# cbg-ethz/metMHN

Measured on AMD Instinct MI355X. Metric: full-cohort log-lik+grad evals/sec at n=20 events; kronvec HBM GB/s, higher is better.
Workload: dtype f64

## Files before the change

metmhn_amd/csrc/engine.hip:

```cpp
#include <algorithm>
#include <chrono>
#include <cmath>
#include <cstdio>
#include <cstdlib>
#include <cstring>
#include <string>
#include <vector>

#include "../../include/metmhn_amd.h"
#include "host.h"
#include "comm.h"
#include "plan.h"
#include "sampler.h"

namespace mmhn {

static thread_local std::string g_err;

struct CListDev {
  DevArr<CItem> items;
  DevArr<int> deps;
};
struct StagedDev {
  DevArr<int> pats, paired, probs;
// ... 14 lines not shown
};

struct Config {
  PlanCfg plan;
  bool zero_copy = true;
  bool poison = false;
  bool force_timing = false;
  bool coop_fault = false;
  int coop_wgs = 0;
  bool coop = true;
  long long sim_chunk = 1ll << 26;
  int stream_blocks = 256 * 8;
  bool trace_host = false;
  Config() {
    plan.use_jacobi = env_is("MMHN_SOLVER", "jacobi");
    plan.psolve_min = (int)env_int("MMHN_PSOLVE_MIN", plan.psolve_min);
    plan.wsolve_min = (int)env_int("MMHN_WSOLVE_MIN", env_set("MMHN_PSOLVE_MIN") ? plan.psolve_min : plan.wsolve_min);
    plan.wsolve_mode = (int)env_int("MMHN_WSOLVE", plan.wsolve_mode);
    plan.wsolve_wgs = (int)env_int("MMHN_WSOLVE_WGS", plan.wsolve_wgs);
    plan.prep_split_max = (int)env_int("MMHN_PREP_SPLIT", plan.prep_split_max);
    plan.pcl_per = std::max(1, (int)env_int("MMHN_PCL_PER", plan.pcl_per));
    plan.small_path = env_flag("MMHN_SMALL", plan.small_path);
    zero_copy = env_flag("MMHN_ZEROCOPY", zero_copy);
    poison = env_flag("MMHN_POISON", poison);
    force_timing = env_flag("MMHN_TIME_KERNELS", force_timing);
    coop_fault = env_flag("MMHN_COOP_FAULT", coop_fault);
    coop_wgs = (int)env_int("MMHN_COOP_WGS", coop_wgs);
    coop = env_flag("MMHN_COOP", coop);
    sim_chunk = std::max(1ll, env_int("MMHN_SIM_CHUNK", sim_chunk));
    stream_blocks = (int)env_int("MMHN_STREAM_BLOCKS", stream_blocks);
    trace_host = env_set("MMHN_TRACE_HOST");
  }
};

struct EngineBase {
  virtual ~EngineBase() = default;
  int dtype = 0;
  int device = 0;
  hipStream_t stream = nullptr;
  Config cfg;
};

template <typename T>
struct PList {
  const Desc* d; const int2* map; int ntiles; int maxk; long long vec;
  const int2* lmap; const std::vector<int>* lof; const T* tab;
  const CList* cl = nullptr;
  const CListDev* dcl = nullptr;
  int kslot = MMHN_K_OTHER_SOLVE;
};

template <typename... K>
static void raise_lds(size_t bytes, K... kernels) {
  for (const void* k : {reinterpret_cast<const void*>(kernels)...})
    HIPCHECK(hipFuncSetAttribute(k, hipFuncAttributeMaxDynamicSharedMemorySize, (int)bytes));
}

template <typename T>
struct Engine : EngineBase {
  using PList = mmhn::PList<T>;
  int n = 0, N = 0;
  DevArr<Params<T>> d_par;
  Params<T>* h_par = nullptr;
  void* h_par_dev = nullptr;
  DevArr<uint16_t> d_perm;
  DevArr<int> d_lvl;
  std::vector<int8_t> dat;
  long long n_pat = 0;
  int n_cols = 0;
  double n_em = 0;
  std::vector<Batch> batches;
  std::vector<BatchDev> dev;
  DevArr<T> pi, lidgJ, qJ, rhsJ, rhsS, pS, lidgS, qS, seedS, GS, dots, bmJ, bmS, tabJ, tabS;
  DevArr<T> piM, qM;
  DevArr<T> zarena;
  struct View { T* p = nullptr; } GJ, DJ, Abuf;
  int pi_owner = -1, qJ_owner = -1;
  DevArr<double> lp, out, sums, abi_sums, redbuf;
  DevArr<JLink<T>> links;
  double* h_abi = nullptr;
  double* h_abi_dev = nullptr;
  hipStream_t side[3] = {};
  hipEvent_t ev_fork[3] = {}, ev_join[3] = {};
  bool small_forked[2] = {false, false}, fork_recorded[2] = {false, false};
  DevArr<CoopCtl> coop_ctl;
  DevArr<unsigned> coop_flags[2];
  unsigned coop_epoch = 0;
  int coop_slot = 0;
  int cur_lane = 0;
  unsigned* h_abort = nullptr;
  unsigned* h_abort_dev = nullptr;
  bool coop_used = false;
  bool coop_alone = false;
  bool sums_pending = false;
  std::chrono::steady_clock::time_point sums_t0, sums_issued;
  int sums_len = 0;
  int pack_mode = 0;
  double pack_a = 0, pack_b = 0;
  double* pack_dst = nullptr;
  bool packed_in_eval = false;
  double reduce_flag = 0.0, reduce_flag_sum = 0.0;
  bool flag_pending = false;
  ncclComm_t comm = nullptr;
  int comm_rank = 0, comm_size = 1;
  bool time_kernels = true;
  mmhn_counters cnt{};
  std::vector<std::pair<hipEvent_t, hipEvent_t>> ev_pool;
  size_t ev_used = 0;
  std::vector<double> ev_bytes;
  std::vector<int> ev_slot;

  static long long zarena_elems(long long nJ, long long asize, int N) { return up4(3 * nJ * N * N) + up4(3 * nJ * N) + up4(asize); }
  static long long zclear_elems(const Batch& b, int N) { return zarena_elems((long long)b.dJ.size(), b.aclr, N); }

  Engine(int dev_id, int n_mut) : n(n_mut), N(n_mut + 1) {
    device = dev_id;
    cnt.comm_rank = -1;
    REQUIRE(n_mut >= 1 && n_mut < MAXN, "n_mut must be in [1, 31]");
    DevGuard guard(device);
    HIPCHECK(hipStreamCreateWithFlags(&stream, hipStreamNonBlocking));
    d_par.alloc(NPSET);
    HIPCHECK(hipHostMalloc(reinterpret_cast<void**>(&h_par), NPSET * sizeof(Params<T>), hipHostMallocDefault));
    HIPCHECK(hipHostGetDevicePointer(&h_par_dev, h_par, 0));
    static_assert(sizeof(Params<T>) % sizeof(uint4) == 0, "parameter block: whole 16-byte words");
    sums.alloc(2 * stride());
    size_t free_b = 0, total_b = 0;
    HIPCHECK(hipMemGetInfo(&free_b, &total_b));
    cfg.plan.ws_limit = (size_t)(0.7 * (double)free_b);
    hipDeviceProp_t prop;
    HIPCHECK(hipGetDeviceProperties(&prop, device));
    cfg.plan.n_cu = std::max(1, prop.multiProcessorCount);
    {
      std::vector<uint16_t> perm((size_t)(TB + 1) << TB, 0);
      std::vector<int> lvl((size_t)(TB + 1) * (TB + 2), 0);
      for (int t = 0; t <= TB; ++t) {
        int pos = 0;
        for (int l = 0; l <= t; ++l) {
          lvl[(size_t)t * (TB + 2) + l] = pos;
          for (uint32_t x = 0; x < (1u << t); ++x)
            if (popc(x) == l) perm[((size_t)t << TB) + pos++] = (uint16_t)x;
        }
        lvl[(size_t)t * (TB + 2) + t + 1] = pos;
      }
      d_perm.alloc(perm.size());
      d_lvl.alloc(lvl.size());
      HIPCHECK(hipMemcpy(d_perm.p, perm.data(), perm.size() * sizeof(uint16_t), hipMemcpyHostToDevice));
      HIPCHECK(hipMemcpy(d_lvl.p, lvl.data(), lvl.size() * sizeof(int), hipMemcpyHostToDevice));
    }
    raise_lds(wsolve_lds<T>(), &k_wsolve<T, false>, &k_wsolve<T, true>, &k_wsolve<T, false, WCfg<T>::NXT>, &k_wsolve<T, true, WCfg<T>::NXT>);
    raise_lds(wclass_lds<T>(), &k_wclass<T>);
    raise_lds(160 * 1024, &k_spatient2<T>, &k_spatient<T, 1024, 1>);
    raise_lds(150 * 1024,
              &k_csolve<T, false, false>, &k_csolve<T, true, false>, &k_csolve<T, false, true>, &k_csolve<T, true, true>,
              &k_csolve<T, false, false, 4>, &k_csolve<T, true, false, 4>,
              &k_psolve2<T, false, true>, &k_psolve2<T, true, true>, &k_psolve2<T, false, false>, &k_psolve2<T, true, false>,
              &k_tsolve<T, false, false>, &k_tsolve<T, true, false>, &k_tsolve<T, false, true>, &k_tsolve<T, true, true>,
              &k_kv<T, false, 1, false>, &k_kv<T, true, 1, false>, &k_kv<T, false, 1, true>, &k_kv<T, true, 1, true>,
              &k_sweep<T, false>, &k_sweep<T, true>, &k_diag<T>, &k_diag<T, 1024>,
              &k_prep<T, false>, &k_prep<T, true>, &k_prep<T, false, 1024>, &k_grad_rows<T, 1>, &k_grad_rows<T>,
              &k_pclass<T, false>, &k_pclass<T, true>, &k_class_marg<T>);
    coop_ctl.alloc(1);
    HIPCHECK(hipMemset(coop_ctl.p, 0, sizeof(CoopCtl)));
    HIPCHECK(hipHostMalloc(reinterpret_cast<void**>(&h_abort), 64, hipHostMallocDefault));
    HIPCHECK(hipHostGetDevicePointer(reinterpret_cast<void**>(&h_abort_dev), h_abort, 0));
    *h_abort = 0u;
    for (int i = 0; i < 3; ++i) {
      HIPCHECK(hipStreamCreateWithFlags(&side[i], hipStreamNonBlocking));
      HIPCHECK(hipEventCreateWithFlags(&ev_fork[i], hipEventDisableTiming));
      HIPCHECK(hipEventCreateWithFlags(&ev_join[i], hipEventDisableTiming));
    }
  }
  ~Engine() override {
    comm_destroy();
    for (auto& e : ev_pool) { (void)hipEventDestroy(e.first); (void)hipEventDestroy(e.second); }
    for (int i = 0; i < 3; ++i) {
      if (ev_join[i]) (void)hipEventDestroy(ev_join[i]);
      if (ev_fork[i]) (void)hipEventDestroy(ev_fork[i]);
      if (side[i]) (void)hipStreamDestroy(side[i]);
    }
    if (h_par) (void)hipHostFree(h_par);
    if (h_abi) (void)hipHostFree(h_abi);
    if (h_abort) (void)hipHostFree(h_abort);
    if (stream) (void)hipStreamDestroy(stream);
    stream = nullptr;
  }
  int stride() const { return 1 + N * N + 2 * N; }

  void build_params(const double* lt, const double* ldp, const double* ldm, bool upload = true) {
    REQUIRE(!sums_pending, "an evaluation begun with mmhn_cohort_sums_begin has not been collected (its parameter upload may still be in flight)");
    std::vector<double> eth((size_t)N * N), enp(N, 1.0), enm(N, 1.0);
    for (int e = 0; e < N * N; ++e) eth[e] = std::exp(lt[e]);
    if (ldp) for (int j = 0; j < N; ++j) enp[j] = std::exp(-ldp[j]);
    if (ldm) for (int j = 0; j < N; ++j) enm[j] = std::exp(-ldm[j]);
    for (int s = 0; s < NPSET; ++s) {
      Params<T>& P = h_par[s];
      std::memset(&P, 0, sizeof(P));
      for (int i = 0; i < N; ++i) {
        for (int j = 0; j < N; ++j) {
          double v = eth[i * N + j];
          if (s == PS_PRIM && j == n && i < n) v = 1.0;
          if (s == PS_MET && i != j) v *= enm[j];
          if (s == PS_PRIM && i != j) v *= enp[j];
          P.th[i][j] = (T)v;
        }
        P.baseP[i] = (T)eth[i * N + i];
        P.baseM[i] = i < n ? (T)(eth[i * N + i] * eth[i * N + n]) : (T)0;
        P.dp[i] = (T)(ldp ? std::exp(ldp[i]) : 1.0);
        P.dm[i] = (T)(ldm ? std::exp(ldm[i]) : 1.0);
      }
    }
    if (!upload) return;
    if (cfg.zero_copy) {
      const int nw = (int)(NPSET * sizeof(Params<T>) / sizeof(uint4));
      hipLaunchKernelGGL(k_copy_words, dim3((nw + 255) / 256), dim3(256), 0, stream, static_cast<const uint4*>(h_par_dev),
                         reinterpret_cast<uint4*>(d_par.p), nw);
      HIPCHECK(hipGetLastError());
    } else {
      HIPCHECK(hipMemcpyAsync(d_par.p, h_par, NPSET * sizeof(Params<T>), hipMemcpyHostToDevice, stream));
    }
  }

  size_t sweep_lds(int maxk) const { return DESC_PAD + ((size_t)(1 << TB) + 2 * (size_t)std::max(maxk, 1) * 64) * sizeof(T); }
  void prep(const Desc* descs, int nprob, T* tab, bool joint = false, int maxkc = 0) {
    if (nprob == 0) return;
    const int parts = maxkc > 9 ? 1 << std::min(maxkc - 9, 5) : 1;
    if (joint && nprob <= cfg.plan.prep_split_max) hipLaunchKernelGGL((k_prep<T, true>), dim3(nprob, 4 * parts), dim3(BLOCK), prep_lds<T>(N), stream, descs, d_par.p, tab);
    else if (nprob >= 256) hipLaunchKernelGGL((k_prep<T, false, 1024>), dim3(nprob), dim3(1024), prep_lds<T>(N), stream, descs, d_par.p, tab);
    else hipLaunchKernelGGL((k_prep<T, false>), dim3(nprob), dim3(BLOCK), prep_lds<T>(N), stream, descs, d_par.p, tab);
    HIPCHECK(hipGetLastError());
  }

  void launch_sweep(bool tr, const Desc* descs, const int2* map, int ntiles, int maxk, const T* p, T* y,
                    const T* lidg, const T* rhs, int rhs_mode, const T* scal, double alg_bytes, const T* tab) {
    if (ntiles == 0) return;
    const size_t lds = sweep_lds(maxk);
    auto launch = [&]() {
      if (tr)
        hipLaunchKernelGGL((k_sweep<T, true>), dim3(ntiles), dim3(KSB), lds, stream, descs, map, d_par.p, p, y,
                           lidg, rhs, rhs_mode, scal, std::max(maxk, 1), tab);
      else
        hipLaunchKernelGGL((k_sweep<T, false>), dim3(ntiles), dim3(KSB), lds, stream, descs, map, d_par.p, p, y,
                           lidg, rhs, rhs_mode, scal, std::max(maxk, 1), tab);
    };
    if (alg_bytes > 0) { timed(MMHN_K_OTHER_SOLVE, alg_bytes, launch); return; }
    launch();
    HIPCHECK(hipGetLastError());
  }
  void launch_kv(bool tr, const Desc* descs, const int2* map, int ntiles, int maxk, const T* p, T* y, const T* tab, const T* hxt,
                 const int* zmap = nullptr, const T* lidg = nullptr, const T* rhs = nullptr) {
    if (ntiles == 0) return;
    const size_t lds = DESC_PAD + ((size_t)(1 << TB) + 2 * (size_t)maxk * 64 + 32) * sizeof(T);
#define KV_ARGS dim3(ntiles), dim3(KSB), lds, stream, descs, map, ntiles, p, y, tab, hxt, maxk, zmap, lidg, rhs
    if (lidg) {
      if (tr) hipLaunchKernelGGL((k_kv<T, true, 1, true>), KV_ARGS);
      else hipLaunchKernelGGL((k_kv<T, false, 1, true>), KV_ARGS);
    } else {
      if (tr) hipLaunchKernelGGL((k_kv<T, true, 1, false>), KV_ARGS);
// ... 248 lines not shown
    links.alloc(std::max<size_t>(mnJ, 1));
    tabJ.alloc(mtJ); tabS.alloc(mtS);
    pi_owner = qJ_owner = -1;
    rhsS.alloc(mvS); pS.alloc(mvS); lidgS.alloc(mvS); qS.alloc(mvS);
    seedS.alloc(mnS);
    GS.alloc(mnS * N * N); zarena.alloc(mZ);
    dots.alloc(2 * mp); bmJ.alloc(mnJ * 64); bmS.alloc(mnS * 64);
    lp.alloc(mp); out.alloc(mp * stride()); redbuf.alloc(((mp + red_per((int)mp) - 1) / red_per((int)mp)) * 2 * (size_t)stride());
  }

  void small_fork(int which) {
    HIPCHECK(hipEventRecord(ev_fork[which], stream));
    fork_recorded[which] = true;
  }
  void small_classes(const Batch& b, int which, bool grad) {
    const BatchDev& db = dev[b.id];
    const int n0 = (int)b.sp_list[which][0].size(), n1 = (int)b.sp_list[which][1].size(), n2 = (int)b.sp_list[which][2].size();
    const int np0 = which ? (int)b.sp_list[2][0].size() : 0, np1 = which ? (int)b.sp_list[2][1].size() : 0;
    const int mk0 = spatient_class_maxk(0), mk1 = which ? b.mk1p : spatient_class_maxk(1), mk2 = spatient_class_maxk(2);
    const bool on_side = which == 0 ? (n0 + n1 + n2 > 0) : n2 > 0;
    hipStream_t sd = side[which];
    if (on_side) {
      if (!fork_recorded[which]) HIPCHECK(hipEventRecord(ev_fork[which], stream));
      HIPCHECK(hipStreamWaitEvent(sd, ev_fork[which], 0));
    }
    fork_recorded[which] = false;
#define SP_TAIL db.pats.p, db.dS.p, d_par.p, d_perm.p, d_lvl.p, db.dJ.p, db.wd.p, pi.p, links.p, pS.p, qS.p, GS.p, bmS.p, dots.p, lp.p
    auto big_class = [&]() {
      if (!n2) return;
      const size_t lds = (spatient_lds<T>(N, mk2) + 15) / 16 * 16;
      hipLaunchKernelGGL((k_spatient<T, 1024, 1>), dim3(n2), dim3(1024), lds, sd, db.sp_list[which][2].p, n2, SP_TAIL, mk2, N, grad ? 1 : 0);
      HIPCHECK(hipGetLastError());
    };
    big_class();
    if (n0 + n1 + np0 + np1) {
      const size_t s0 = (spatient_lds<T>(N, mk0) + 15) / 16 * 16, s1 = (spatient_lds<T>(N, mk1) + 15) / 16 * 16;
      const size_t lds = std::max(s0 * SP_PPB0, n1 + np1 ? s1 * (np1 ? 2 : 1) : 0) + 64;
      const int nblk = (n0 + SP_PPB0 - 1) / SP_PPB0 + n1 + (np0 + SP_PPB0 / 2 - 1) / (SP_PPB0 / 2) + np1;
      hipLaunchKernelGGL((k_spatient2<T>), dim3(nblk), dim3(256), lds, which == 0 ? sd : stream,
                         db.sp_list[which][0].p, n0, mk0, db.sp_list[which][1].p, n1, mk1,
                         db.sp_list[2][0].p, np0, db.sp_list[2][1].p, np1, SP_TAIL, N, grad ? 1 : 0);
      HIPCHECK(hipGetLastError());
    }
#undef SP_TAIL
    if (on_side) HIPCHECK(hipEventRecord(ev_join[which], sd));
    small_forked[which] = on_side;
  }
  void small_join(int which) {
    if (small_forked[which]) HIPCHECK(hipStreamWaitEvent(stream, ev_join[which], 0));
    small_forked[which] = false;
  }

  void evaluate(const double* lt, const double* ldp, const double* ldm, bool grad, double* host_sums,
                double* host_out) {
    REQUIRE(!sums_pending, "an evaluation begun with mmhn_cohort_sums_begin has not been collected");
    auto t0 = std::chrono::steady_clock::now();
    const int st = stride();
    small_forked[0] = small_forked[1] = fork_recorded[0] = fork_recorded[1] = false;
    bool head_done = false;
    if (cfg.zero_copy && !batches.empty()) {
      build_params(lt, ldp, ldm, false);
      const Batch& b0 = batches.front();
      long long nz = grad && !b0.dJ.empty() ? zclear_elems(b0, N) * (long long)sizeof(T) / 16 : 0;
      const bool fill_here = nz <= (32ll << 20) / 16;
      if (!fill_here) nz = 0;
      const int nw = (int)(NPSET * sizeof(Params<T>) / sizeof(uint4));
      const long long need = std::max<long long>(std::max<long long>(nw, 2 * st), nz);
      const int nblk = (int)std::min<long long>((need + 255) / 256, 4096);
      hipLaunchKernelGGL(k_begin_eval, dim3(nblk), dim3(256), 0, stream, static_cast<const uint4*>(h_par_dev),
                         reinterpret_cast<uint4*>(d_par.p), nw, sums.p, 2 * st, reinterpret_cast<uint4*>(zarena.p), nz);
      HIPCHECK(hipGetLastError());
      head_done = fill_here;
    } else {
      build_params(lt, ldp, ldm);
      HIPCHECK(hipMemsetAsync(sums.p, 0, 2 * st * sizeof(double), stream));
    }
    for (const Batch& b : batches) {
      const BatchDev& db = dev[b.id];
      const int npat = (int)b.pats.size(), nJ = (int)b.dJ.size(), nS = (int)b.dS.size();
      const int tJ = (int)b.mapJ.size();
      const PList LJ{db.dJ.p, db.mapJ.p, tJ, b.maxkJ, b.vecJ, db.lmapJ.p, &b.lofJ, tabJ.p};
      const bool fused_small = b.has_small;
      coop_alone = b.stg[0].empty();
      auto staged_fwd = [&](int w) {
        const Staged& g = b.stg[w];
        const StagedDev& dg = db.stg[w];
        if (g.empty()) return;
        const int nG = (int)g.pats.size(), tG = (int)g.map.size();
        const PList LG{db.dS.p, dg.map.p, tG, g.maxk, b.vecS, dg.lmap.p, &g.lof, tabS.p, g.cl, dg.cl};
        hipLaunchKernelGGL((k_staged_init<T>), dim3(nG), dim3(BLOCK), 0, stream, db.pats.p, db.dS.p, rhsS.p, GS.p, bmS.p, N, grad ? 1 : 0, dg.pats.p);
        HIPCHECK(hipGetLastError());
        if (g.probs.size() >= 256)
          hipLaunchKernelGGL((k_prep<T, false, 1024>), dim3((unsigned)g.probs.size()), dim3(1024), prep_lds<T>(N), stream, db.dS.p, d_par.p, tabS.p, dg.probs.p);
        else
          hipLaunchKernelGGL((k_prep<T, false>), dim3((unsigned)g.probs.size()), dim3(BLOCK), prep_lds<T>(N), stream, db.dS.p, d_par.p, tabS.p, dg.probs.p);
        HIPCHECK(hipGetLastError());
        if (!g.paired.empty()) {
          hipLaunchKernelGGL((k_gather_marg<T>), dim3((unsigned)g.paired.size(), 2, g.maxk > 10 ? 8 : 1), dim3(BLOCK), 0, stream,
                             db.pats.p, db.dJ.p, db.dS.p, d_par.p, pi.p, rhsS.p, links.p, dg.paired.p, db.wd.p);
          HIPCHECK(hipGetLastError());
        }
        launch_diag(db.dS.p, dg.map.p, tG, nullptr, lidgS.p, nullptr, KD_LIDG);
        solve(false, LG, pS.p, lidgS.p, rhsS.p, 0, nullptr);
        hipLaunchKernelGGL((k_seeds<T>), dim3((nG + 255) / 256), dim3(256), 0, stream, db.pats.p, nG, db.dS.p,
                           d_par.p, pS.p, seedS.p, lp.p, dg.pats.p);
        HIPCHECK(hipGetLastError());
      };
      auto staged_adj = [&](int w) {
        const Staged& g = b.stg[w];
        const StagedDev& dg = db.stg[w];
        if (g.empty()) return;
        const int tG = (int)g.map.size();
        const PList LG{db.dS.p, dg.map.p, tG, g.maxk, b.vecS, dg.lmap.p, &g.lof, tabS.p, g.cl, dg.cl};
        solve(true, LG, qS.p, lidgS.p, nullptr, 1, seedS.p);
        launch_grad_rows(db.dS.p, (int)g.probs.size(), g.maxk, nullptr, pS.p, qS.p, GS.p, GK_S, dg.grc);
        if (g.kind2) {
          hipLaunchKernelGGL((k_bit_marg<T>), dim3(tG), dim3(BLOCK), 0, stream, db.dS.p, dg.map.p, d_par.p, pS.p, qS.p, bmS.p);
          HIPCHECK(hipGetLastError());
        }
      };
      time_kernels = cfg.force_timing || b.vecJ + b.vecS >= (1ll << 26);
      const long long gjs = (long long)nJ * N * N;
      GJ.p = zarena.p;
      DJ.p = GJ.p + up4(3 * gjs);
      Abuf.p = DJ.p + up4(3ll * nJ * N);
      if (grad && nJ && !(head_done && &b == &batches.front())) zero(zarena.p, zclear_elems(b, N));
      if (grad && nJ && cfg.poison) poison_fill(Abuf.p + b.aclr, b.asize - b.aclr);
      prep(db.dJ.p, nJ, tabJ.p, true, b.maxkcJ);
      bool own_forked = false;
      if (!b.stg[0].empty() && !time_kernels) {
        HIPCHECK(hipEventRecord(ev_fork[2], stream));
        HIPCHECK(hipStreamWaitEvent(side[2], ev_fork[2], 0));
        hipStream_t keep = stream;
        stream = side[2]; cur_lane = 1;
        try {
          staged_fwd(0);
          if (grad) staged_adj(0);
        } catch (...) { stream = keep; cur_lane = 0; throw; }
        stream = keep; cur_lane = 0;
        HIPCHECK(hipEventRecord(ev_join[2], side[2]));
        own_forked = true;
      }
      if (fused_small) small_fork(0);
      if (!cfg.plan.use_jacobi && nJ) {
        if (pi_owner != b.id) { zero(pi.p + b.offT, b.vecJ - b.offT); pi_owner = b.id; }
        if (grad && qJ_owner != b.id) { zero(qJ.p + b.offT, b.vecJ - b.offT); qJ_owner = b.id; }
        if (cfg.poison && b.offT > 0) {
          HIPCHECK(hipMemsetAsync(pi.p, 0xFF, (size_t)b.offT * sizeof(T), stream));
          if (grad) HIPCHECK(hipMemsetAsync(qJ.p, 0xFF, (size_t)b.offT * sizeof(T), stream));
        }
      }
      if (cfg.plan.use_jacobi) {
        launch_diag(db.dJ.p, db.mapJ.p, tJ, nullptr, lidgJ.p, nullptr, KD_LIDG);
        solve(false, LJ, pi.p, lidgJ.p, nullptr, 2, nullptr);
      } else {
        psolve(false, b, pi.p, 2);
      }
      if (fused_small) small_classes(b, 0, grad);
      if (fused_small) small_classes(b, 1, grad);
      if (!own_forked) staged_fwd(0);
      staged_fwd(1);
      if (grad) {
        if (!own_forked) staged_adj(0);
        staged_adj(1);
        small_join(1);
        if (nJ) {
          if (cfg.plan.use_jacobi) zero(rhsJ.p, b.vecJ);
          for (int part = 0; part < 2 && !b.stg[1].paired.empty(); ++part) {
            if (b.stg[1].paired.size() >= 256)
              hipLaunchKernelGGL((k_scatter_marg<T, 1024>), dim3((unsigned)b.stg[1].paired.size()), dim3(1024), 0, stream, db.pats.p, db.dJ.p,
                                 db.dS.p, d_par.p, qS.p, rhsS.p, cfg.plan.use_jacobi ? rhsJ.p : nullptr, dots.p, part, db.stg[1].paired.p);
            else
            hipLaunchKernelGGL((k_scatter_marg<T>), dim3((unsigned)b.stg[1].paired.size()), dim3(BLOCK), 0, stream, db.pats.p, db.dJ.p,
                               db.dS.p, d_par.p, qS.p, rhsS.p, cfg.plan.use_jacobi ? rhsJ.p : nullptr, dots.p, part, db.stg[1].paired.p);
            HIPCHECK(hipGetLastError());
          }
          if (cfg.plan.use_jacobi) solve(true, LJ, qJ.p, lidgJ.p, rhsJ.p, 0, nullptr);
          else psolve(true, b, qJ.p, 3);
          if (!cfg.plan.use_jacobi) {
            const double mbytes = (double)b.vecJ * sizeof(T);
            timed(MMHN_K_PCLASS, mbytes, [&]() {
              if (b.wdirect) {
                const int nW = (int)b.wd.size();
                hipLaunchKernelGGL((k_wclass<T>), dim3((unsigned)std::min(nW, cfg.plan.n_cu)), dim3(WROWS), wclass_lds<T>(), stream, db.dJ.p, db.wd.p, nW, pi.p, qJ.p, Abuf.p);
              }
              if (!b.pcl.empty())
                hipLaunchKernelGGL((k_pclass<T, true>), dim3((unsigned)b.pcl.size()), dim3(CMB), PC_LDS_ELEMS * sizeof(T), stream, db.dJ.p, db.wd.p, pi.p, qJ.p, Abuf.p, db.pcl.p);
              else if ((int)b.wd.size() < nJ || !b.wdirect)
                hipLaunchKernelGGL((k_pclass<T, false>), dim3(nJ), dim3(CMB), PC_LDS_ELEMS * sizeof(T), stream, db.dJ.p, db.wd.p, pi.p, qJ.p, Abuf.p);
            });
            if (!b.mapX.empty())
              hipLaunchKernelGGL((k_class_marg<T>), dim3((unsigned)b.mapX.size()), dim3(CMB), 2 * sizeof(T) << TB, stream,
                                 db.dJ.p, db.mapX.p, pi.p, qJ.p, Abuf.p);
          } else {
            hipLaunchKernelGGL((k_class_marg<T>), dim3(tJ), dim3(CMB), 2 * sizeof(T) << TB, stream, db.dJ.p,
                               db.mapJ.p, pi.p, qJ.p, Abuf.p);
          }
          HIPCHECK(hipGetLastError());
          if (b.pcl.empty()) {
            hipLaunchKernelGGL((k_eq_flows<T>), dim3(nJ), dim3(BLOCK), 0, stream, db.dJ.p, db.wd.p, pi.p, qJ.p, Abuf.p);
            HIPCHECK(hipGetLastError());
          }
          launch_grad_rows(db.dJ.p, nJ, b.maxkcJ, Abuf.p, nullptr, nullptr, GJ.p, -1, db.grcJ, DJ.p, gjs);
        }
      }
      if (fused_small) { small_join(0); small_join(1); }
      if (own_forked) HIPCHECK(hipStreamWaitEvent(stream, ev_join[2], 0));
      const AsmArgs<T> aa{db.pats.p, db.dJ.p, db.dS.p, d_par.p, GS.p, GJ.p, gjs, dots.p, DJ.p, (long long)nJ * N, bmS.p, lp.p, N,
                          grad ? 1 : 0};
      const int nelem = grad ? st : 1;
      hipLaunchKernelGGL((k_finalize<T>), dim3(npat), dim3(BLOCK), 0, stream, aa, out.p);
      HIPCHECK(hipGetLastError());
      {
        const int per = red_per(npat), nchunk = (npat + per - 1) / per;
        const dim3 cols((nelem + BLOCK - 1) / BLOCK);
        hipLaunchKernelGGL(k_reduce_rows, dim3(cols.x, nchunk), dim3(BLOCK), 0, stream, db.pats.p, npat, per, out.p, st, nelem, redbuf.p);
        HIPCHECK(hipGetLastError());
        if (pack_mode && &b == &batches.back()) {
          hipLaunchKernelGGL(k_reduce_parts_pack, dim3((st + BLOCK - 1) / BLOCK), dim3(BLOCK), 0, stream, redbuf.p, st, nelem, nchunk,
                             sums.p, pack_mode, N, pack_a, pack_b, pack_dst);
          packed_in_eval = true;
        } else {
          hipLaunchKernelGGL(k_reduce_parts, dim3(cols.x, 2), dim3(BLOCK), 0, stream, redbuf.p, st, nelem, nchunk, sums.p);
        }
        HIPCHECK(hipGetLastError());
      }
      if (host_out) {
        std::vector<double> tmp((size_t)npat * st);
        HIPCHECK(hipMemcpyAsync(tmp.data(), out.p, tmp.size() * sizeof(double), hipMemcpyDeviceToHost, stream));
        HIPCHECK(hipStreamSynchronize(stream));
        check_abort();
        for (int i = 0; i < npat; ++i)
          std::memcpy(host_out + (size_t)b.pats[i].row * st, tmp.data() + (size_t)i * st, st * sizeof(double));
      }
    }
    time_kernels = true;
    if (host_sums) {
      std::vector<double> hs(2 * st);
      HIPCHECK(hipMemcpyAsync(hs.data(), sums.p, hs.size() * sizeof(double), hipMemcpyDeviceToHost, stream));
      HIPCHECK(hipStreamSynchronize(stream));
      check_abort();
      std::memcpy(host_sums, hs.data(), hs.size() * sizeof(double));
      finish_eval(t0);
    }
  }
  void reset_counters() {
    const int r = cnt.comm_ranks, k = cnt.comm_rank;
    cnt = mmhn_counters{};
    cnt.comm_ranks = r; cnt.comm_rank = k;
  }
  void finish_eval(std::chrono::steady_clock::time_point t0) {
    collect_events();
    cnt.eval_ms += std::chrono::duration<double, std::milli>(std::chrono::steady_clock::now() - t0).count();
    cnt.evals += 1;
  }

  void cohort_sums_begin(const double* lt, const double* ldp, const double* ldm, bool grad, const double* w_combined = nullptr) {
    REQUIRE(!sums_pending, "mmhn_cohort_sums_begin: the previous evaluation has not been collected");
    sums_t0 = std::chrono::steady_clock::now();
    const int full = 4 + 2 * N * N + 3 * N;
    const int total = w_combined ? stride() : full;
    abi_sums.alloc(full);
    if (!h_abi) {
      HIPCHECK(hipHostMalloc(reinterpret_cast<void**>(&h_abi), (size_t)full * sizeof(double), hipHostMallocDefault));
      HIPCHECK(hipHostGetDevicePointer(reinterpret_cast<void**>(&h_abi_dev), h_abi, 0));
    }
    double* packed = (cfg.zero_copy && !comm) ? h_abi_dev : abi_sums.p;
    pack_mode = w_combined ? 2 : 1;
    pack_a = w_combined ? *w_combined : (double)n_em; pack_b = w_combined ? reduce_flag : (double)n_pat; pack_dst = packed;
    packed_in_eval = false;
    struct Unset { int& m; ~Unset() { m = 0; } } unset{pack_mode};
    evaluate(lt, ldp, ldm, grad, nullptr, nullptr);
    if (!packed_in_eval) {
      if (w_combined) hipLaunchKernelGGL(k_pack_wsums, dim3(2), dim3(256), 0, stream, sums.p, N, *w_combined, packed, reduce_flag);
      else hipLaunchKernelGGL(k_pack_sums, dim3(2), dim3(256), 0, stream, sums.p, N, n_em, (double)n_pat, packed);
      HIPCHECK(hipGetLastError());
    }
    const int moved = total + (w_combined ? 1 : 0);
    if (comm) RCCLCHECK(rccl().AllReduce(abi_sums.p, abi_sums.p, (size_t)moved, ncclFloat64, ncclSum, comm, stream));
    if (packed == abi_sums.p) HIPCHECK(hipMemcpyAsync(h_abi, abi_sums.p, moved * sizeof(double), hipMemcpyDeviceToHost, stream));
    flag_pending = w_combined != nullptr;
    reduce_flag = 0.0;
    sums_issued = std::chrono::steady_clock::now();
    sums_pending = true;
    sums_len = total;
  }
  void cohort_sums_end(double* o, int expect_len) {
// ... 623 lines not shown
```

metmhn_amd/csrc/marg.h:

```cpp
#pragma once
#include "common.h"

namespace mmhn {


template <typename T>
__device__ __forceinline__ T obs_const(const Desc& dj, const Params<T>& P, int part) {
  T c = part == 0 ? P.dp[dj.N - 1] : P.dm[dj.N - 1];
  for (int b = 0; b < dj.k; ++b)
    if (dj.cls[b] == (part == 0 ? CP : CM)) c *= (part == 0 ? P.dp[dj.ev[b]] : P.dm[dj.ev[b]]);
  return c;
}

template <typename T>
__global__ __launch_bounds__(BLOCK) void k_gather_marg(const PatRec* __restrict__ pats,
                                                       const Desc* __restrict__ dJ,
                                                       const Desc* __restrict__ dS,
                                                       const Params<T>* __restrict__ par,
                                                       const T* __restrict__ pi, T* rhsS, JLink<T>* links,
                                                       const int* __restrict__ paired, const WDesc* __restrict__ wds) {
  __shared__ Desc djs;
  const PatRec pr = pats[paired[blockIdx.x]];
  const int part = blockIdx.y;
  const int sp = part == 0 ? pr.s[0] : pr.s[1];
  if (pr.j < 0) return;
  const bool writes_link = threadIdx.x == 0 && blockIdx.z == 0;
  if (sp < 0) {
    if (writes_link) { links[pr.j].soff[part] = -1; links[pr.j].sk[part] = 0; links[pr.j].cst[part] = 0; }
    return;
  }
  load_desc(&djs, dJ + pr.j);
  const int ksS = dS[sp].k;
  const long long offS = dS[sp].off;
  __syncthreads();
  const Desc& dj = djs;
  const uint32_t fixed = (part == 0 ? dj.maskP : dj.maskM) | (1u << dj.seedbit);
  const uint32_t free_ = part == 0 ? dj.maskM : dj.maskP;
  const uint32_t half = 1u << (ksS - 1);
  const T c = obs_const(dj, par[PS_THETA], part);
  if (writes_link) { links[pr.j].soff[part] = offS; links[pr.j].sk[part] = ksS; links[pr.j].cst[part] = c; }
  const bool free_is_row = dj.wl >= 0 && (wds[dj.wl].majP != 0) == (part == 1);
  for (uint32_t e = blockIdx.z * BLOCK + threadIdx.x; e < half; e += gridDim.z * BLOCK) {
    const long long x = dj.wl >= 0 ? wpos_marg<T>(wds[dj.wl], dj.k, free_is_row, e) : (long long)(pdep32(e, free_) | fixed);
    rhsS[offS + e] = 0;
    rhsS[offS + half + e] = c * pi[dj.off + x];
  }
}

template <typename T, int KB = BLOCK>
__global__ __launch_bounds__(KB) void k_scatter_marg(const PatRec* __restrict__ pats,
                                                        const Desc* __restrict__ dJ,
                                                        const Desc* __restrict__ dS,
                                                        const Params<T>* __restrict__ par,
                                                        const T* __restrict__ qS,
                                                        const T* __restrict__ rhsS, T* rhsJ,
                                                        T* dots, int part, const int* __restrict__ plist) {
  __shared__ T red[KB];
  const int pat = plist ? plist[blockIdx.x] : (int)blockIdx.x;
  const PatRec pr = pats[pat];
  if (pr.j < 0 || pr.s[part] < 0) return;
  const Desc& dj = dJ[pr.j];
  const Desc& ds = dS[pr.s[part]];
  const uint32_t fixed = (part == 0 ? dj.maskP : dj.maskM) | (1u << dj.seedbit);
  const uint32_t free_ = part == 0 ? dj.maskM : dj.maskP;
  const uint32_t half = 1u << (ds.k - 1);
  const T c = obs_const(dj, par[PS_THETA], part);
  T dot = 0;
  for (uint32_t e = threadIdx.x; e < half; e += KB) {
    const uint32_t x = pdep32(e, free_) | fixed;
    const T qv = qS[ds.off + half + e];
    if (rhsJ) rhsJ[dj.off + x] += c * qv;
    dot += qv * rhsS[ds.off + half + e];
  }
  red[threadIdx.x] = dot;
  __syncthreads();
  for (int s = KB / 2; s > 0; s >>= 1) {
    if ((int)threadIdx.x < s) red[threadIdx.x] += red[threadIdx.x + s];
    __syncthreads();
  }
  if (threadIdx.x == 0) dots[2 * pat + part] = red[0];
}

template <typename T>
__global__ __launch_bounds__(BLOCK) void k_staged_init(const PatRec* __restrict__ pats, const Desc* __restrict__ dS, T* rhsS,
                                                       T* GS, T* bmS, int N, int with_grad, const int* __restrict__ plist) {
  const PatRec pr = pats[plist[blockIdx.x]];
  for (int part = 0; part < 2; ++part) {
    const int sp = pr.s[part];
    if (sp < 0) continue;
    if (with_grad) {
      for (int e = threadIdx.x; e < N * N; e += BLOCK) GS[(long long)sp * N * N + e] = T(0);
      if (threadIdx.x < 64) bmS[(long long)sp * 64 + threadIdx.x] = T(0);
    }
    if (pr.kind <= 2 && part == 0) {
      const long long off = dS[sp].off, V = 1ll << dS[sp].k;
      for (long long e = threadIdx.x; e < V; e += BLOCK) rhsS[off + e] = e == 0 ? e0_scale<T>() : T(0);
    }
  }
}

template <typename T>
__global__ void k_seeds(const PatRec* __restrict__ pats, int npat, const Desc* __restrict__ dS,
                        const Params<T>* __restrict__ par, const T* __restrict__ pS, T* seedS,
                        double* lp, const int* __restrict__ plist) {
  const int ii = blockIdx.x * blockDim.x + threadIdx.x;
  if (ii >= npat) return;
  const int i = plist ? plist[ii] : ii;
  const PatRec pr = pats[i];
  if (pr.kind == 4) return;
  T full = 0;
  for (int part = 0; part < 2; ++part)
    if (pr.s[part] >= 0) {
      const Desc& ds = dS[pr.s[part]];
      full += pS[ds.off + (1ll << ds.k) - 1];
    }
  for (int part = 0; part < 2; ++part)
    if (pr.s[part] >= 0) seedS[pr.s[part]] = T(1) / full;
  double l = log((double)full) - log((double)e0_scale<T>());
  if (pr.kind == 2) {
    const Desc& ds = dS[pr.s[0]];
    const Params<T>& P = par[PS_THETA];
    double dr = (double)P.dm[ds.N - 1];
    for (int b = 0; b < ds.k; ++b)
      if (b != ds.seedbit) dr *= (double)P.dm[ds.ev[b]];
    l += log(dr);
  }
  lp[i] = l;
}

}
```

metmhn_amd/csrc/small.h:

```cpp
#pragma once
#include "kernels.h"

namespace mmhn {

constexpr int SP_NCLASS = 3;
constexpr int SP_PPB0 = 4;
__host__ __device__ inline int spatient_class_maxk(int c) { return c == 0 ? 6 : c == 1 ? 9 : TB; }
__host__ __device__ inline int spatient_lstride(int maxk) { return maxk < 6 ? 1 << maxk : 64; }
__host__ __device__ inline int spatient_rows(int maxk) { return maxk > 6 ? 1 << (maxk - 6) : 1; }

template <typename T>
__host__ __device__ inline size_t spatient_lds(int N, int maxk) {
  return ((size_t)N * (spatient_lstride(maxk) + spatient_rows(maxk) + 16 + 1) + 4 * 64 + 2 * 16 + ((size_t)3 << maxk) + 64) * sizeof(T) +
         (64 + TB + 2) * sizeof(int) + 8 + DESC_PAD + (sizeof(uint16_t) << maxk);
}

template <typename T, int SPB, int PPB, bool PAIR = false>
__device__ __forceinline__ void spatient_body(const int* __restrict__ plist, int npl, const PatRec* __restrict__ pats, const Desc* __restrict__ dS,
                                              const Params<T>* __restrict__ par,
                                              const uint16_t* __restrict__ perm, const int* __restrict__ lvl,
                                              const Desc* __restrict__ dJ, const WDesc* __restrict__ wds, const T* __restrict__ pi, JLink<T>* __restrict__ links,
                                              T* __restrict__ pS, T* __restrict__ qS,
                                              T* __restrict__ GS, T* __restrict__ bmS, T* __restrict__ dots,
                                              double* __restrict__ lp, int maxk, int N, int with_grad, int block) {
// ... 113 lines not shown
    sync();
  };
  auto solve = [&](const Desc& d, T* y, bool tr, auto rhs) {
    const int k = d.k;
    const uint32_t V = 1u << k, full = V - 1u;
    for (uint32_t x = tid; x < V; x += SPB) y[x] = rhs(x);
    sync();
    auto state = [&](uint32_t x) {
      T z = y[x];
      if (!tr) {
        for (uint32_t m = x; m; m &= m - 1) {
          const int b = __ffs(m) - 1;
          const uint32_t xs = x ^ (1u << b);
          z += Lc[lev[b] * LS + (xs & 63u)] * Uc[lev[b] * RS + (xs >> 6)] * y[xs];
        }
      } else {
        for (uint32_t m = ~x & full; m; m &= m - 1) {
          const int b = __ffs(m) - 1;
          z += Lc[lev[b] * LS + (x & 63u)] * Uc[lev[b] * RS + (x >> 6)] * y[x | (1u << b)];
        }
      }
      y[x] = LID[x] * z;
    };
    const int ns = kwalk >= 0 ? kwalk : k;
    for (int s = 0; s <= ns; ++s) {
      const int level = tr ? k - s : s;
      if (SPB == 64) {
        if ((uint32_t)tid < V && __popc((uint32_t)tid) == level) state((uint32_t)tid);
      } else if (s <= k) {
        for (int idx = loff[level] + tid; idx < loff[level + 1]; idx += SPB) state(pml[idx]);
      }
      sync();
    }
  };

  struct Marg { T c; uint32_t fixed, free_, half; long long joff; int wl, kj; bool free_is_row; };
  auto marg_of = [&](int part, int k) -> Marg {
    const Desc* dj = dJ + pr.j;
    const Params<T>& PT = par[PS_THETA];
    const int kj = dj->k;
    sync();
    if (tid < 32) {
      T f = 1;
      if (tid < kj && dj->cls[tid] == (part == 0 ? CP : CM)) f = part == 0 ? PT.dp[dj->ev[tid]] : PT.dm[dj->ev[tid]];
      red[tid] = f;
    }
    sync();
    T c = part == 0 ? PT.dp[N - 1] : PT.dm[N - 1];
    for (int b = 0; b < kj; ++b) c *= red[b];
    sync();
    Marg m;
    m.c = c;
    m.fixed = (part == 0 ? dj->maskP : dj->maskM) | (1u << dj->seedbit);
    m.free_ = part == 0 ? dj->maskM : dj->maskP;
    m.half = 1u << (k - 1);
    m.joff = dj->off;
    m.wl = dj->wl; m.kj = kj;
    m.free_is_row = m.wl >= 0 && (wds[m.wl].majP != 0) == (part == 1);
    return m;
  };
  auto marg_rhs = [&](const Marg& m, uint32_t x) -> T {
    if (x < m.half) return T(0);
    if (m.wl >= 0) return m.c * pi[m.joff + wpos_marg<T>(wds[m.wl], m.kj, m.free_is_row, x - m.half)];
    return m.c * pi[m.joff + (pdep32(x - m.half, m.free_) | m.fixed)];
  };
  Marg mg0{}, mg1{};

  STAMP_DECL;
  STAMP_START;
  T full_score = 0;
  for (int part = 0; part < 2; ++part) {
    const int sp = part == 0 ? ps0 : ps1;
    if (sp < 0 || (PAIR && part != mypart)) continue;
    setup(dS[sp]);
    STAMP(0);
    const Desc& d = dsh;
    const bool own = pr.kind <= 2;
    Marg mg{};
    if (!own) {
      mg = marg_of(part, d.k);
      if (part == 0) mg0 = mg; else mg1 = mg;
      if (tid == 0) { links[pr.j].soff[part] = d.off; links[pr.j].sk[part] = d.k; links[pr.j].cst[part] = mg.c; }
    }
    const bool stash = !PAIR && part == 1 && ps0 >= 0;
    T* yv = stash ? Qv : P0;
    solve(d, yv, false, [&](uint32_t x) { return own ? (x == 0 ? e0_scale<T>() : T(0)) : marg_rhs(mg, x); });
    full_score += yv[(1u << d.k) - 1u];
    if (stash) for (uint32_t x = tid; x < (1u << d.k); x += SPB) pS[d.off + x] = yv[x];
    STAMP(1);
  }
  if (pr.kind == 3 && !PAIR && tid == 0) {
    if (ps0 < 0) { links[pr.j].soff[0] = -1; links[pr.j].sk[0] = 0; links[pr.j].cst[0] = 0; }
    if (ps1 < 0) { links[pr.j].soff[1] = -1; links[pr.j].sk[1] = 0; links[pr.j].cst[1] = 0; }
  }
  if (PAIR) {
    if (tid == 0) xch[pslot] = full_score;
    __syncthreads();
    full_score = xch[pslot & ~1] + xch[pslot | 1];
  }
  const T seed = T(1) / full_score;
  if (tid == 0 && !(PAIR && mypart == 1)) {
    double l = log((double)full_score) - log((double)e0_scale<T>());
    if (pr.kind == 2) {
      const Desc& d = dsh;
      const Params<T>& P = par[PS_THETA];
      double dr = (double)P.dm[N - 1];
      for (int b = 0; b < d.k; ++b) if (b != d.seedbit) dr *= (double)dml[b];
      l += log(dr);
    }
    lp[pat] = l;
  }
  STAMP(2);
  if (!with_grad) { STAMP_FLUSH(0); return; }

  const int nparts = (ps0 >= 0) + (ps1 >= 0);
  for (int part = 0; part < 2; ++part) {
    const int sp = part == 0 ? ps0 : ps1;
    if (sp < 0 || (PAIR && part != mypart)) continue;
    if (nparts == 2 && !PAIR) setup(dS[sp]);
    const Desc& d = dsh;
    const int k = d.k;
    const uint32_t V = 1u << k, last = V - 1u;
    solve(d, Qv, true, [&](uint32_t x) { return x == last ? seed : T(0); });
    STAMP(3);
    if (!PAIR && part == 1 && ps0 >= 0) {
      sync();
      for (uint32_t x = tid; x < V; x += SPB) P0[x] = pS[d.off + x];
      sync();
    }
    const T* p = P0;
    if (pr.kind == 3) {
      T* qg = qS + d.off;
      const Marg& mg = part == 0 ? mg0 : mg1;
      const uint32_t half = V >> 1;
      T dot = 0;
      for (uint32_t x = tid; x < V; x += SPB) {
        const T qv = Qv[x];
        qg[x] = qv;
        if (x >= half) dot += qv * marg_rhs(mg, x);
      }
      dot = wave_sum_dpp(dot);
      if (lane == 0) red[w] = dot;
      sync();
      if (tid == 0) { T t = 0; for (int v = 0; v < SPW; ++v) t += red[v]; dots[2 * pat + part] = t; }
    }
    if (pr.kind == 2) {
      T* bm = bmS + (long long)sp * 64;
      const Params<T>& P0 = par[d.pset];
      T accA[TB], accB[TB];
#pragma unroll
      for (int b = 0; b < TB; ++b) { accA[b] = 0; accB[b] = 0; }
      for (uint32_t x = tid; x < V; x += SPB) {
        const uint32_t lo = x & 63u, ro = x >> 6;
        const bool sbit = d.seedbit >= 0 && ((x >> d.seedbit) & 1u);
        const T pq = p[x] * Qv[x];
        const T vA = sbit ? T(0) : pq * LA[lo] * UA[ro], vB = sbit ? pq * LB[lo] * UB[ro] * P0.dm[n] : T(0);
#pragma unroll
        for (int b = 0; b < TB; ++b) if (b < k && ((x >> b) & 1u)) { accA[b] += vA; accB[b] += vB; }
      }
      sync();
      T* part_ = LID;
#pragma unroll
      for (int b = 0; b < TB; ++b) {
        if (b < k) {
          const T a = wave_sum_dpp(accA[b]), bb = wave_sum_dpp(accB[b]);
          if (lane == 0) { part_[(w * 2 + 0) * TB + b] = a; part_[(w * 2 + 1) * TB + b] = bb; }
        }
      }
      sync();
      if (tid < 64) {
        const int ww = tid >> 5, b = tid & 31;
        T m = 0;
        if (b < k) for (int v = 0; v < SPW; ++v) m += part_[(v * 2 + ww) * TB + b];
        bm[ww * 32 + b] = m;
      }
    }
    STAMP(4);
    T* G = GS + (long long)sp * N * N;
    if (SPW == 1) {
      const int i = lane & 31, h = lane >> 5;
      const bool rowok = i < N;
      const int slot = rowok ? d.bitP[i] : -1;
      const int kt = k > 0 ? k - 1 : 0;
      const uint32_t Vh = k > 0 ? V >> 1 : 1u, hs = h && k > 0 ? Vh : 0u;
      T tot = 0, acc[6];
#pragma unroll
      for (int l = 0; l < 6; ++l) acc[l] = 0;
      if (rowok && !(h && k == 0)) {
        const T ui = Uc[i * RS];
        const uint32_t sb = slot >= 0 ? 1u << slot : 0u;
#pragma unroll 4
        for (uint32_t Sl = 0; Sl < Vh; ++Sl) {
          const uint32_t S = Sl | hs;
          const T pv = p[S], q0 = Qv[S], q1 = Qv[S | sb], lc = Lc[i * LS + S];
          T a = -pv * q0;
          if (slot >= 0) a += pv * q1;
          const T f = (S & sb) ? T(0) : lc * ui * a;
          tot += f;
#pragma unroll
          for (int l = 0; l < 5; ++l) if ((Sl >> l) & 1u) acc[l] += f;
        }
      }
      const T tup = __shfl_down(tot, 32);
      T aup[5];
#pragma unroll
      for (int l = 0; l < 5; ++l) aup[l] = __shfl_down(acc[l], 32);
      if (rowok && h == 0) {
        if (k > 0) {
// ... 94 lines not shown
```

Before: 22.41.

## Overlap staged-class prep on side stream and reorder small-patient solve parts

Splits staged-class work into pre, forward, adjoint and gradient-row phases. The prep and diagonal kernels for staged group 1 are forked onto a side stream so they overlap with joint-chain work, and group-1 grad rows are deferred until after the joint gradient. Scatter-marg launches for both parts are merged into one 2D grid when Jacobi is not used. The small-patient kernel now runs the backward pass in reverse part order, so the last forward solution stays in LDS and one stash and reload of pS is avoided. The cost is extra event synchronisation, and stream ordering and part-ordering logic become harder to get right.

```diff
diff --git a/metmhn_amd/csrc/engine.hip b/metmhn_amd/csrc/engine.hip
--- a/metmhn_amd/csrc/engine.hip
+++ b/metmhn_amd/csrc/engine.hip
@@ -120,6 +120,7 @@
   double* h_abi_dev = nullptr;
   hipStream_t side[3] = {};
   hipEvent_t ev_fork[3] = {}, ev_join[3] = {};
+  hipEvent_t ev_pre[2] = {};
   bool small_forked[2] = {false, false}, fork_recorded[2] = {false, false};
   DevArr<CoopCtl> coop_ctl;
   DevArr<unsigned> coop_flags[2];
@@ -207,10 +208,12 @@
       HIPCHECK(hipEventCreateWithFlags(&ev_fork[i], hipEventDisableTiming));
       HIPCHECK(hipEventCreateWithFlags(&ev_join[i], hipEventDisableTiming));
     }
+    for (hipEvent_t& e : ev_pre) HIPCHECK(hipEventCreateWithFlags(&e, hipEventDisableTiming));
   }
   ~Engine() override {
     comm_destroy();
     for (auto& e : ev_pool) { (void)hipEventDestroy(e.first); (void)hipEventDestroy(e.second); }
+    for (hipEvent_t e : ev_pre) if (e) (void)hipEventDestroy(e);
     for (int i = 0; i < 3; ++i) {
       if (ev_join[i]) (void)hipEventDestroy(ev_join[i]);
       if (ev_fork[i]) (void)hipEventDestroy(ev_fork[i]);
@@ -625,12 +628,11 @@
       const PList LJ{db.dJ.p, db.mapJ.p, tJ, b.maxkJ, b.vecJ, db.lmapJ.p, &b.lofJ, tabJ.p};
       const bool fused_small = b.has_small;
       coop_alone = b.stg[0].empty();
-      auto staged_fwd = [&](int w) {
+      auto staged_pre = [&](int w) {
         const Staged& g = b.stg[w];
         const StagedDev& dg = db.stg[w];
         if (g.empty()) return;
         const int nG = (int)g.pats.size(), tG = (int)g.map.size();
-        const PList LG{db.dS.p, dg.map.p, tG, g.maxk, b.vecS, dg.lmap.p, &g.lof, tabS.p, g.cl, dg.cl};
         hipLaunchKernelGGL((k_staged_init<T>), dim3(nG), dim3(BLOCK), 0, stream, db.pats.p, db.dS.p, rhsS.p, GS.p, bmS.p, N, grad ? 1 : 0, dg.pats.p);
         HIPCHECK(hipGetLastError());
         if (g.probs.size() >= 256)
@@ -638,12 +640,19 @@
         else
           hipLaunchKernelGGL((k_prep<T, false>), dim3((unsigned)g.probs.size()), dim3(BLOCK), prep_lds<T>(N), stream, db.dS.p, d_par.p, tabS.p, dg.probs.p);
         HIPCHECK(hipGetLastError());
+        launch_diag(db.dS.p, dg.map.p, tG, nullptr, lidgS.p, nullptr, KD_LIDG);
+      };
+      auto staged_fwd = [&](int w) {
+        const Staged& g = b.stg[w];
+        const StagedDev& dg = db.stg[w];
+        if (g.empty()) return;
+        const int nG = (int)g.pats.size(), tG = (int)g.map.size();
+        const PList LG{db.dS.p, dg.map.p, tG, g.maxk, b.vecS, dg.lmap.p, &g.lof, tabS.p, g.cl, dg.cl};
         if (!g.paired.empty()) {
           hipLaunchKernelGGL((k_gather_marg<T>), dim3((unsigned)g.paired.size(), 2, g.maxk > 10 ? 8 : 1), dim3(BLOCK), 0, stream,
                              db.pats.p, db.dJ.p, db.dS.p, d_par.p, pi.p, rhsS.p, links.p, dg.paired.p, db.wd.p);
           HIPCHECK(hipGetLastError());
         }
-        launch_diag(db.dS.p, dg.map.p, tG, nullptr, lidgS.p, nullptr, KD_LIDG);
         solve(false, LG, pS.p, lidgS.p, rhsS.p, 0, nullptr);
         hipLaunchKernelGGL((k_seeds<T>), dim3((nG + 255) / 256), dim3(256), 0, stream, db.pats.p, nG, db.dS.p,
                            d_par.p, pS.p, seedS.p, lp.p, dg.pats.p);
@@ -656,6 +665,12 @@
         const int tG = (int)g.map.size();
         const PList LG{db.dS.p, dg.map.p, tG, g.maxk, b.vecS, dg.lmap.p, &g.lof, tabS.p, g.cl, dg.cl};
         solve(true, LG, qS.p, lidgS.p, nullptr, 1, seedS.p);
+      };
+      auto staged_rows = [&](int w) {
+        const Staged& g = b.stg[w];
+        const StagedDev& dg = db.stg[w];
+        if (g.empty()) return;
+        const int tG = (int)g.map.size();
         launch_grad_rows(db.dS.p, (int)g.probs.size(), g.maxk, nullptr, pS.p, qS.p, GS.p, GK_S, dg.grc);
         if (g.kind2) {
           hipLaunchKernelGGL((k_bit_marg<T>), dim3(tG), dim3(BLOCK), 0, stream, db.dS.p, dg.map.p, d_par.p, pS.p, qS.p, bmS.p);
@@ -667,6 +682,16 @@
       GJ.p = zarena.p;
       DJ.p = GJ.p + up4(3 * gjs);
       Abuf.p = DJ.p + up4(3ll * nJ * N);
+      const bool pre_forked = !b.stg[1].empty();
+      if (pre_forked) {
+        HIPCHECK(hipEventRecord(ev_pre[0], stream));
+        HIPCHECK(hipStreamWaitEvent(side[2], ev_pre[0], 0));
+        hipStream_t keep = stream;
+        stream = side[2];
+        try { staged_pre(1); } catch (...) { stream = keep; throw; }
+        stream = keep;
+        HIPCHECK(hipEventRecord(ev_pre[1], side[2]));
+      }
       if (grad && nJ && !(head_done && &b == &batches.front())) zero(zarena.p, zclear_elems(b, N));
       if (grad && nJ && cfg.poison) poison_fill(Abuf.p + b.aclr, b.asize - b.aclr);
       prep(db.dJ.p, nJ, tabJ.p, true, b.maxkcJ);
@@ -677,8 +702,9 @@
         hipStream_t keep = stream;
         stream = side[2]; cur_lane = 1;
         try {
+          staged_pre(0);
           staged_fwd(0);
-          if (grad) staged_adj(0);
+          if (grad) { staged_adj(0); staged_rows(0); }
         } catch (...) { stream = keep; cur_lane = 0; throw; }
         stream = keep; cur_lane = 0;
         HIPCHECK(hipEventRecord(ev_join[2], side[2]));
@@ -701,21 +727,25 @@
       }
       if (fused_small) small_classes(b, 0, grad);
       if (fused_small) small_classes(b, 1, grad);
-      if (!own_forked) staged_fwd(0);
+      if (!own_forked) { staged_pre(0); staged_fwd(0); }
+      if (pre_forked) HIPCHECK(hipStreamWaitEvent(stream, ev_pre[1], 0));
       staged_fwd(1);
       if (grad) {
-        if (!own_forked) staged_adj(0);
+        if (!own_forked) { staged_adj(0); staged_rows(0); }
         staged_adj(1);
         small_join(1);
         if (nJ) {
           if (cfg.plan.use_jacobi) zero(rhsJ.p, b.vecJ);
-          for (int part = 0; part < 2 && !b.stg[1].paired.empty(); ++part) {
+          const int nsc = b.stg[1].paired.empty() ? 0 : cfg.plan.use_jacobi ? 2 : 1;
+          for (int part = 0; part < nsc; ++part) {
+            const dim3 g((unsigned)b.stg[1].paired.size(), cfg.plan.use_jacobi ? 1 : 2);
+            const int parg = cfg.plan.use_jacobi ? part : -1;
             if (b.stg[1].paired.size() >= 256)
-              hipLaunchKernelGGL((k_scatter_marg<T, 1024>), dim3((unsigned)b.stg[1].paired.size()), dim3(1024), 0, stream, db.pats.p, db.dJ.p,
-                                 db.dS.p, d_par.p, qS.p, rhsS.p, cfg.plan.use_jacobi ? rhsJ.p : nullptr, dots.p, part, db.stg[1].paired.p);
+              hipLaunchKernelGGL((k_scatter_marg<T, 1024>), g, dim3(1024), 0, stream, db.pats.p, db.dJ.p,
+                                 db.dS.p, d_par.p, qS.p, rhsS.p, cfg.plan.use_jacobi ? rhsJ.p : nullptr, dots.p, parg, db.stg[1].paired.p);
             else
-            hipLaunchKernelGGL((k_scatter_marg<T>), dim3((unsigned)b.stg[1].paired.size()), dim3(BLOCK), 0, stream, db.pats.p, db.dJ.p,
-                               db.dS.p, d_par.p, qS.p, rhsS.p, cfg.plan.use_jacobi ? rhsJ.p : nullptr, dots.p, part, db.stg[1].paired.p);
+              hipLaunchKernelGGL((k_scatter_marg<T>), g, dim3(BLOCK), 0, stream, db.pats.p, db.dJ.p,
+                                 db.dS.p, d_par.p, qS.p, rhsS.p, cfg.plan.use_jacobi ? rhsJ.p : nullptr, dots.p, parg, db.stg[1].paired.p);
             HIPCHECK(hipGetLastError());
           }
           if (cfg.plan.use_jacobi) solve(true, LJ, qJ.p, lidgJ.p, rhsJ.p, 0, nullptr);
@@ -746,6 +776,7 @@
           }
           launch_grad_rows(db.dJ.p, nJ, b.maxkcJ, Abuf.p, nullptr, nullptr, GJ.p, -1, db.grcJ, DJ.p, gjs);
         }
+        staged_rows(1);
       }
       if (fused_small) { small_join(0); small_join(1); }
       if (own_forked) HIPCHECK(hipStreamWaitEvent(stream, ev_join[2], 0));
diff --git a/metmhn_amd/csrc/marg.h b/metmhn_amd/csrc/marg.h
--- a/metmhn_amd/csrc/marg.h
+++ b/metmhn_amd/csrc/marg.h
@@ -54,8 +54,9 @@
                                                         const Params<T>* __restrict__ par,
                                                         const T* __restrict__ qS,
                                                         const T* __restrict__ rhsS, T* rhsJ,
-                                                        T* dots, int part, const int* __restrict__ plist) {
+                                                        T* dots, int part_arg, const int* __restrict__ plist) {
   __shared__ T red[KB];
+  const int part = part_arg < 0 ? (int)blockIdx.y : part_arg;
   const int pat = plist ? plist[blockIdx.x] : (int)blockIdx.x;
   const PatRec pr = pats[pat];
   if (pr.j < 0 || pr.s[part] < 0) return;
diff --git a/metmhn_amd/csrc/small.h b/metmhn_amd/csrc/small.h
--- a/metmhn_amd/csrc/small.h
+++ b/metmhn_amd/csrc/small.h
@@ -219,11 +219,10 @@
       if (part == 0) mg0 = mg; else mg1 = mg;
       if (tid == 0) { links[pr.j].soff[part] = d.off; links[pr.j].sk[part] = d.k; links[pr.j].cst[part] = mg.c; }
     }
-    const bool stash = !PAIR && part == 1 && ps0 >= 0;
-    T* yv = stash ? Qv : P0;
-    solve(d, yv, false, [&](uint32_t x) { return own ? (x == 0 ? e0_scale<T>() : T(0)) : marg_rhs(mg, x); });
-    full_score += yv[(1u << d.k) - 1u];
-    if (stash) for (uint32_t x = tid; x < (1u << d.k); x += SPB) pS[d.off + x] = yv[x];
+    const bool stash = !PAIR && part == 0 && ps1 >= 0;
+    solve(d, P0, false, [&](uint32_t x) { return own ? (x == 0 ? e0_scale<T>() : T(0)) : marg_rhs(mg, x); });
+    full_score += P0[(1u << d.k) - 1u];
+    if (stash) for (uint32_t x = tid; x < (1u << d.k); x += SPB) pS[d.off + x] = P0[x];
     STAMP(1);
   }
   if (pr.kind == 3 && !PAIR && tid == 0) {
@@ -251,16 +250,17 @@
   if (!with_grad) { STAMP_FLUSH(0); return; }
 
   const int nparts = (ps0 >= 0) + (ps1 >= 0);
-  for (int part = 0; part < 2; ++part) {
+  for (int pp = 0; pp < 2; ++pp) {
+    const int part = (nparts == 2 && !PAIR) ? 1 - pp : pp;
     const int sp = part == 0 ? ps0 : ps1;
     if (sp < 0 || (PAIR && part != mypart)) continue;
-    if (nparts == 2 && !PAIR) setup(dS[sp]);
+    if (nparts == 2 && !PAIR && part == 0) setup(dS[sp]);
     const Desc& d = dsh;
     const int k = d.k;
     const uint32_t V = 1u << k, last = V - 1u;
     solve(d, Qv, true, [&](uint32_t x) { return x == last ? seed : T(0); });
     STAMP(3);
-    if (!PAIR && part == 1 && ps0 >= 0) {
+    if (!PAIR && part == 0 && ps1 >= 0) {
       sync();
       for (uint32_t x = tid; x < V; x += SPB) P0[x] = pS[d.off + x];
       sync();
```

New measurement: 22.43 (median of 2 runs). Within noise of the previous version (+0.1%).
